# facebookresearch/momentum

Measured on NVIDIA H100. Metric: GN iterations/sec (batched 72-joint IK), higher is better.
Workload: dtype f32

## Files before the change

momentum_b200/csrc/ik_chol_sched.cuh:

```cuda
#pragma once

#include <cmath>
#include <cstring>

#include "ik_types.h"

#include <vector_types.h>

namespace mb2 {

struct CholSchedDev {
  int32_t n, nPad, numTileCols, numTiles, numLevels;
  const int32_t* blob;
  int32_t blobInts;
  const int32_t* perm;
  const int32_t* pos;
  const int32_t* tileIdTable;
  const int32_t* tileRow;
  const int32_t* tileCol;
  const int32_t* diagTile;
  const int32_t* levelColStart;
  const int32_t* levelCols;
  const int32_t* levelPanelStart;
  const int32_t* panelTile;
  const int32_t* panelDiag;
  const int32_t* levelTaskStart;
  const int32_t* taskDst;
  const int32_t* taskPairStart;
  const int32_t* pairA;
  const int32_t* pairB;
  const int32_t* levelVTaskStart;
  const int32_t* vtaskRow;
  const int32_t* vtaskSrcStart;
  const int32_t* vsrcTile;
  const int32_t* vsrcCol;
  const int32_t* colPanelStart;
  const int32_t* colPanelTile;
  const int32_t* colPanelRow;
  const int32_t* levelOrderStart8;
  const int32_t* taskOrder8;
  const int32_t* levelOrderStart16;
  const int32_t* taskOrder16;
  const int32_t* tileInfo;
};
MB2_HD CholSchedDev rebaseSchedule(const CholSchedDev& S, const int32_t* newBlob) {
  CholSchedDev R = S;
  const int32_t* o = S.blob;
  R.blob = newBlob;
#define MB2_RB(f) R.f = newBlob + (S.f - o);
  MB2_RB(perm) MB2_RB(pos) MB2_RB(tileIdTable) MB2_RB(tileRow) MB2_RB(tileCol) MB2_RB(diagTile) MB2_RB(levelColStart) MB2_RB(levelCols)
  MB2_RB(levelPanelStart) MB2_RB(panelTile) MB2_RB(panelDiag) MB2_RB(levelTaskStart) MB2_RB(taskDst) MB2_RB(taskPairStart) MB2_RB(pairA) MB2_RB(pairB)
  MB2_RB(levelVTaskStart) MB2_RB(vtaskRow) MB2_RB(vtaskSrcStart) MB2_RB(vsrcTile) MB2_RB(vsrcCol) MB2_RB(colPanelStart) MB2_RB(colPanelTile)
  MB2_RB(colPanelRow) MB2_RB(levelOrderStart8) MB2_RB(taskOrder8) MB2_RB(levelOrderStart16) MB2_RB(taskOrder16) MB2_RB(tileInfo)
#undef MB2_RB
  return R;
}

MB2_HD int tileSlotOffset(int lane) { return (lane ^ (lane >> 3)) << 2; }
MB2_HD int tileIdx(int r, int c) {
  const int lane = ((r & 7) << 2) | ((c & 7) >> 1);
  return ((c >> 3) << 7) + ((lane ^ (lane >> 3)) << 2) + (((r >> 3) << 1) | (c & 1));
}
MB2_HD int fragRow(int lane, int e) { return (lane >> 2) + 8 * (e >> 1); }
MB2_HD int fragCol(int lane, int h, int e) { return 8 * h + 2 * (lane & 3) + (e & 1); }
MB2_HD void tileLoadFrag(const float* tile, int lane, float d[2][4]) {
  const int so = tileSlotOffset(lane);
#if defined(__CUDA_ARCH__)
  const float4 v0 = *reinterpret_cast<const float4*>(tile + so), v1 = *reinterpret_cast<const float4*>(tile + 128 + so);
  d[0][0] = v0.x; d[0][1] = v0.y; d[0][2] = v0.z; d[0][3] = v0.w; d[1][0] = v1.x; d[1][1] = v1.y; d[1][2] = v1.z; d[1][3] = v1.w;
#else
  for (int h = 0; h < 2; ++h) for (int e = 0; e < 4; ++e) d[h][e] = tile[128 * h + so + e];
#endif
}
MB2_HD void tileStoreFrag(float* tile, int lane, const float d[2][4]) {
  const int so = tileSlotOffset(lane);
#if defined(__CUDA_ARCH__)
  *reinterpret_cast<float4*>(tile + so) = make_float4(d[0][0], d[0][1], d[0][2], d[0][3]);
  *reinterpret_cast<float4*>(tile + 128 + so) = make_float4(d[1][0], d[1][1], d[1][2], d[1][3]);
#else
  for (int h = 0; h < 2; ++h) for (int e = 0; e < 4; ++e) tile[128 * h + so + e] = d[h][e];
#endif
}

MB2_HD float cholPadElement(float v, int info, int r, int c) {
  const int vI = info & 0xFF, vJ = (info >> 8) & 0xFF, diag = (info >> 16) & 1;
  if (r < vI && c < vJ) return v;
  return (diag && r == c) ? 1.f : 0.f;
}
MB2_HD int tmaBoxIdx(int c, int r) { return c * 16 + ((((r >> 2) ^ ((c >> 1) & 3)) << 2) | (r & 3)); }
MB2_HD void cholConvertBox(float* tile, int info, int lane) {
  float v[2][4];
#pragma unroll
  for (int h = 0; h < 2; ++h)
#pragma unroll
    for (int e = 0; e < 4; ++e) {
      const int r = fragRow(lane, e), c = fragCol(lane, h, e);
      const bool mirror = ((info >> 16) & 1) != 0 && c > r;
      v[h][e] = cholPadElement(tile[mirror ? tmaBoxIdx(r, c) : tmaBoxIdx(c, r)], info, r, c);
    }
#if defined(__CUDA_ARCH__)
  __syncwarp();
#endif
  tileStoreFrag(tile, lane, v);
}

MB2_HD float tf32High(float x) {
#if defined(__CUDA_ARCH__)
  return __uint_as_float((__float_as_uint(x) + 0x1000u) & 0xFFFFE000u);
#else
  uint32_t u;
  std::memcpy(&u, &x, 4);
  u = (u + 0x1000u) & 0xFFFFE000u;
  float r;
  std::memcpy(&r, &u, 4);
  return r;
#endif
}
#if defined(__CUDA_ARCH__)
__device__ __forceinline__ void mmaTf32K8(float d[4], float a0, float a1, float a2, float a3, float b0, float b1) {
  asm volatile("mma.sync.aligned.m16n8k8.row.col.f32.tf32.tf32.f32 {%0, %1, %2, %3}, {%4, %5, %6, %7}, {%8, %9}, {%0, %1, %2, %3};"
               : "+f"(d[0]), "+f"(d[1]), "+f"(d[2]), "+f"(d[3])
               : "r"(__float_as_uint(a0)), "r"(__float_as_uint(a1)), "r"(__float_as_uint(a2)), "r"(__float_as_uint(a3)), "r"(__float_as_uint(b0)),
                 "r"(__float_as_uint(b1)));
}
__device__ __forceinline__ void mma3xTf32Step(float d[2][4], float small[2][4], float a0, float a1, float a2, float a3, float b00, float b01, float b10, float b11) {
  const float a0h = tf32High(a0), a1h = tf32High(a1), a2h = tf32High(a2), a3h = tf32High(a3);
  const float b00h = tf32High(b00), b01h = tf32High(b01), b10h = tf32High(b10), b11h = tf32High(b11);
  const float a0l = a0 - a0h, a1l = a1 - a1h, a2l = a2 - a2h, a3l = a3 - a3h;
  const float b00l = b00 - b00h, b01l = b01 - b01h, b10l = b10 - b10h, b11l = b11 - b11h;
  mmaTf32K8(small[0], a0l, a1l, a2l, a3l, b00h, b01h); mmaTf32K8(small[1], a0l, a1l, a2l, a3l, b10h, b11h);
  mmaTf32K8(small[0], a0h, a1h, a2h, a3h, b00l, b01l); mmaTf32K8(small[1], a0h, a1h, a2h, a3h, b10l, b11l);
  float t0[4] = {0.f, 0.f, 0.f, 0.f}, t1[4] = {0.f, 0.f, 0.f, 0.f};
  mmaTf32K8(t0, a0h, a1h, a2h, a3h, b00h, b01h); mmaTf32K8(t1, a0h, a1h, a2h, a3h, b10h, b11h);
#pragma unroll
  for (int e = 0; e < 4; ++e) { d[0][e] += t0[e]; d[1][e] += t1[e]; }
}
#endif
MB2_HD void mma3xEmulate(float& d, float& small, const float av[8], const float bv[8]) {
  float lo = 0.f, mid = 0.f, hi = 0.f;
  for (int k = 0; k < 8; ++k) {
    const float ah = tf32High(av[k]), bh = tf32High(bv[k]), al = av[k] - ah, bl = bv[k] - bh;
    lo += al * bh; mid += ah * bl; hi += ah * bh;
  }
  small += lo + mid;
  d += hi;
}

MB2_HD void gramTilePairs(const float* strips, int oa0, int ob0, int oa1, int ob1, int lane, float d[2][4], float small[2][4]) {
  const float* A0 = strips + oa0;
  const float* B0 = strips + ob0;
  const float* A1 = strips + oa1;
  const float* B1 = strips + ob1;
#if defined(__CUDA_ARCH__)
  mma3xTf32Step(d, small, A0[lane], A0[32 + lane], A1[lane], A1[32 + lane], B0[lane], B1[lane], B0[32 + lane], B1[32 + lane]);
#else
  for (int h = 0; h < 2; ++h)
    for (int e = 0; e < 4; ++e) {
      const int r = fragRow(lane, e), c = fragCol(lane, h, e);
      float av[8], bv[8];
      for (int k = 0; k < 8; ++k) { av[k] = k < 4 ? A0[4 * r + k] : A1[4 * r + k - 4]; bv[k] = k < 4 ? B0[4 * c + k] : B1[4 * c + k - 4]; }
      mma3xEmulate(d[h][e], small[h][e], av, bv);
    }
#endif
}
MB2_HD int4 tableRecord4(const int32_t* p) {
#if defined(__CUDA_ARCH__)
  return *reinterpret_cast<const int4*>(p);
#else
  int4 r; r.x = p[0]; r.y = p[1]; r.z = p[2]; r.w = p[3];
  return r;
#endif
}
MB2_HD int4 tableRecord4(const uint16_t* p) {
  int4 r;
#if defined(__CUDA_ARCH__)
  const uint2 v = *reinterpret_cast<const uint2*>(p);
  r.x = int(v.x & 0xFFFFu); r.y = int(v.x >> 16); r.z = int(v.y & 0xFFFFu); r.w = int(v.y >> 16);
#else
  r.x = p[0]; r.y = p[1]; r.z = p[2]; r.w = p[3];
#endif
  return r;
}
MB2_HD int2 tableRecord2(const uint16_t* p) {
  int2 r;
#if defined(__CUDA_ARCH__)
  const uint32_t v = *reinterpret_cast<const uint32_t*>(p);
  r.x = int(v & 0xFFFFu); r.y = int(v >> 16);
#else
  r.x = p[0]; r.y = p[1];
#endif
  return r;
}
template <class Q>
MB2_HD void gramTileAccumulate(const float* strips, const Q* quads, int q0, int q1, int lane, float d[2][4]) {
  float small[2][4] = {{0.f, 0.f, 0.f, 0.f}, {0.f, 0.f, 0.f, 0.f}};
  for (int q = q0; q < q1; ++q) {
    const int4 o = tableRecord4(quads + 4 * q);
    gramTilePairs(strips, o.x, o.y, o.z, o.w, lane, d, small);
  }
#pragma unroll
  for (int h = 0; h < 2; ++h)
#pragma unroll
    for (int e = 0; e < 4; ++e) d[h][e] += small[h][e];
}
MB2_HD void gramTileStore(float* tile, const float d[2][4], int info, float lambda, int lane) {
  const int vI = info & 0xFF, vJ = (info >> 8) & 0xFF, diag = (info >> 16) & 1;
  if (vI == 16 && vJ == 16 && !diag) { tileStoreFrag(tile, lane, d); return; }
  float v[2][4];
#pragma unroll
  for (int h = 0; h < 2; ++h)
#pragma unroll
    for (int e = 0; e < 4; ++e) {
      const int r = fragRow(lane, e), c = fragCol(lane, h, e);
      v[h][e] = cholPadElement((diag && r == c) ? d[h][e] + lambda : d[h][e], info, r, c);
    }
  tileStoreFrag(tile, lane, v);
}
MB2_HD void gramVectorTerm(const float* strip, const float* r4, int hl, float& g0, float& g1) {
  const float4 sv = *reinterpret_cast<const float4*>(strip + 4 * hl);
  const float4 rv = *reinterpret_cast<const float4*>(r4);
  g0 += sv.x * rv.x + sv.y * rv.y;
  g1 += sv.z * rv.z + sv.w * rv.w;
}
MB2_HD float gramVectorEntry(const float* strips, const float* resid, const int32_t* colStrip, const int32_t* stripRow, int s0, int s1, int hl) {
  float g0 = 0.f, g1 = 0.f;
  for (int k = s0; k < s1; ++k) {
    const int sidx = colStrip[k];
    gramVectorTerm(strips + size_t(sidx) * 64, resid + stripRow[sidx], hl, g0, g1);
  }
  return g0 + g1;
}
MB2_HD float gramVectorEntry(const float* strips, const float* resid, const uint16_t* colEnt, int s0, int s1, int hl) {
  float g0 = 0.f, g1 = 0.f;
  for (int k = s0; k < s1; ++k) {
    const int2 e = tableRecord2(colEnt + 2 * k);
    gramVectorTerm(strips + e.x, resid + e.y, hl, g0, g1);
  }
  return g0 + g1;
}

MB2_HD void tileLoadRow(const float* tile, int r, float* a) {
#pragma unroll
  for (int j = 0; j < 16; j += 2) {
    const float2 v = *reinterpret_cast<const float2*>(tile + tileIdx(r, j));
    a[j] = v.x; a[j + 1] = v.y;
  }
}
MB2_HD void tileStoreRow(float* tile, int r, const float* a) {
#pragma unroll
  for (int j = 0; j < 16; j += 2) {
    float2 v;
    v.x = a[j]; v.y = a[j + 1];
    *reinterpret_cast<float2*>(tile + tileIdx(r, j)) = v;
  }
}

MB2_HD void cholDiagTile(float* tile, float* y16, int lane, float fallback, int* fail) {
#if defined(__CUDA_ARCH__)
  const int hl = lane & 15;
  const bool isE = lane >= 16;
  float v[16];
#pragma unroll
  for (int k = 0; k < 16; ++k) v[k] = isE ? (k == hl ? 1.f : 0.f) : tile[tileIdx(k, hl)];
  float z = isE ? 0.f : y16[hl], rdSelf = 0.f;
  __syncwarp();
#pragma unroll
  for (int k = 0; k < 16; ++k) {
    float* blk = tile + 32 * (k & 1);
    if (!isE) { blk[hl] = v[k]; blk[16 + hl] = z; }
    __syncwarp();
    float c[16];
#pragma unroll
    for (int g4 = (k >> 2); g4 < 4; ++g4) {
      const float4 q = *reinterpret_cast<const float4*>(blk + 4 * g4);
      c[4 * g4] = q.x; c[4 * g4 + 1] = q.y; c[4 * g4 + 2] = q.z; c[4 * g4 + 3] = q.w;
    }
    float piv = c[k];
    const float zk = blk[16 + k];
    if (!(piv > 0.f)) { piv = fallback; if (lane == k) *fail = 1; }
    float inv;
    asm("rcp.approx.ftz.f32 %0, %1;" : "=f"(inv) : "f"(piv));
    const float rdk = rsqrtf(piv);
    if (lane == k) rdSelf = rdk;
    const float m = v[k] * inv;
    const float tm = (!isE && hl > k) ? m : 0.f;
#pragma unroll
    for (int j = k + 1; j < 16; ++j) v[j] -= m * c[j];
    z -= tm * zk;
    v[k] *= rdk;
  }
  __syncwarp();
  if (!isE) y16[hl] = z * rdSelf;
  else {
#pragma unroll
    for (int i = 0; i < 16; ++i) tile[tileIdx(i, hl)] = v[i];
  }
#else
  if (lane != 0) return;
  float A[16][16], E[16][16], z[16], rd[16];
  for (int l = 0; l < 16; ++l) { for (int k = 0; k < 16; ++k) { A[l][k] = tile[tileIdx(k, l)]; E[k][l] = (k == l) ? 1.f : 0.f; } z[l] = y16[l]; }
  for (int k = 0; k < 16; ++k) {
    float piv = A[k][k];
    if (!(piv > 0.f)) { piv = fallback; *fail = 1; }
    const float inv = 1.f / piv;
    rd[k] = 1.f / sqrtf(piv);
    const float zk = z[k];
    float c[16];
    for (int j = 0; j < 16; ++j) c[j] = A[j][k];
    for (int l = 0; l < 16; ++l) {
      const float m = c[l] * inv;
      for (int j = k + 1; j < 16; ++j) A[l][j] -= m * c[j];
      if (l > k) z[l] -= m * zk;
    }
    for (int l = 0; l < 16; ++l) {
      const float m = E[k][l] * inv;
      for (int j = k + 1; j < 16; ++j) E[j][l] -= m * c[j];
      E[k][l] *= rd[k];
    }
  }
  for (int l = 0; l < 16; ++l) {
    y16[l] = z[l] * rd[l];
    for (int i = 0; i < 16; ++i) tile[tileIdx(i, l)] = E[i][l];
  }
#endif
}

MB2_HD void tileProduct(const float* TA, const float* TB, int lane, float d[2][4], float small[2][4]) {
#if defined(__CUDA_ARCH__)
  const int so = tileSlotOffset(lane);
  const float4 a0 = *reinterpret_cast<const float4*>(TA + so), a1 = *reinterpret_cast<const float4*>(TA + 128 + so);
  const float4 b0 = *reinterpret_cast<const float4*>(TB + so), b1 = *reinterpret_cast<const float4*>(TB + 128 + so);
  mma3xTf32Step(d, small, a0.x, a0.z, a0.y, a0.w, b0.x, b0.y, b0.z, b0.w);
  mma3xTf32Step(d, small, a1.x, a1.z, a1.y, a1.w, b1.x, b1.y, b1.z, b1.w);
#else
  for (int h = 0; h < 2; ++h)
    for (int e = 0; e < 4; ++e) {
      const int r = fragRow(lane, e), c = fragCol(lane, h, e);
      for (int ks = 0; ks < 2; ++ks) {
        float av[8], bv[8];
        for (int k = 0; k < 8; ++k) { av[k] = TA[tileIdx(r, 8 * ks + k)]; bv[k] = TB[tileIdx(c, 8 * ks + k)]; }
        mma3xEmulate(d[h][e], small[h][e], av, bv);
      }
    }
#endif
}

MB2_HD void cholPanelProduct(const float* tile, const float* diagW, int lane, float out[2][4]) {
  float small[2][4];
#pragma unroll
  for (int h = 0; h < 2; ++h)
#pragma unroll
    for (int e = 0; e < 4; ++e) { out[h][e] = 0.f; small[h][e] = 0.f; }
  tileProduct(tile, diagW, lane, out, small);
#pragma unroll
  for (int h = 0; h < 2; ++h)
#pragma unroll
    for (int e = 0; e < 4; ++e) out[h][e] += small[h][e];
}
MB2_HD void cholPanelStore(float* tile, int lane, const float out[2][4]) { tileStoreFrag(tile, lane, out); }

template <class I>
MB2_HD void cholUpdateTile(float* tiles, const I* pairA, const I* pairB, int stride, int p0, int p1, int dst, int lane) {
  float d[2][4], small[2][4];
#pragma unroll
  for (int h = 0; h < 2; ++h)
#pragma unroll
    for (int e = 0; e < 4; ++e) { d[h][e] = 0.f; small[h][e] = 0.f; }
  for (int p = p0; p < p1; ++p)
    tileProduct(tiles + size_t(pairA[p * stride]) * 256, tiles + size_t(pairB[p * stride]) * 256, lane, d, small);
  float* D = tiles + size_t(dst) * 256;
  float v[2][4];
  tileLoadFrag(D, lane, v);
#pragma unroll
  for (int h = 0; h < 2; ++h)
#pragma unroll
    for (int e = 0; e < 4; ++e) v[h][e] -= d[h][e] + small[h][e];
  tileStoreFrag(D, lane, v);
}
MB2_HD void cholUpdateTask(float* tiles, const CholSchedDev& S, int task, int lane) {
  cholUpdateTile(tiles, S.pairA, S.pairB, 1, S.taskPairStart[task], S.taskPairStart[task + 1], S.taskDst[task], lane);
}

template <class I>
MB2_HD void cholVectorRows(const float* tiles, float* y, const I* srcTile, const I* srcCol, int stride, int p0, int p1, int row, int hl) {
  float s0 = 0.f, s1 = 0.f, s2 = 0.f, s3 = 0.f;
  for (int p = p0; p < p1; ++p) {
    float t[16];
    tileLoadRow(tiles + size_t(srcTile[p * stride]) * 256, hl, t);
    const float* yk = y + srcCol[p * stride] * 16;
#pragma unroll
    for (int c = 0; c < 16; c += 4) { s0 += t[c] * yk[c]; s1 += t[c + 1] * yk[c + 1]; s2 += t[c + 2] * yk[c + 2]; s3 += t[c + 3] * yk[c + 3]; }
  }
  y[row * 16 + hl] -= (s0 + s1) + (s2 + s3);
}
MB2_HD void cholVectorTask(const float* tiles, float* y, const CholSchedDev& S, int vtask, int hl) {
  cholVectorRows(tiles, y, S.vsrcTile, S.vsrcCol, 1, S.vtaskSrcStart[vtask], S.vtaskSrcStart[vtask + 1], S.vtaskRow[vtask], hl);
}

template <class I>
MB2_HD void cholBackwardPanels(const float* tiles, float* y, const I* panelTile, const I* panelRow, int stride, int p0, int p1, int K, int diag, int lane) {
#if defined(__CUDA_ARCH__)
  const int g = lane >> 2, t = lane & 3, so = tileSlotOffset(lane);
  float c0 = 0.f, c1 = 0.f, c2 = 0.f, c3 = 0.f;
  for (int p = p0; p < p1; ++p) {
    const float* T = tiles + size_t(panelTile[p * stride]) * 256;
    const float* yi = y + panelRow[p * stride] * 16;
    const float4 v0 = *reinterpret_cast<const float4*>(T + so), v1 = *reinterpret_cast<const float4*>(T + 128 + so);
    const float ya = yi[g], yb = yi[g + 8];
    c0 = fmaf(v0.x, ya, fmaf(v0.z, yb, c0)); c1 = fmaf(v0.y, ya, fmaf(v0.w, yb, c1));
    c2 = fmaf(v1.x, ya, fmaf(v1.z, yb, c2)); c3 = fmaf(v1.y, ya, fmaf(v1.w, yb, c3));
  }
#pragma unroll
  for (int o = 4; o < 32; o <<= 1) {
    c0 += __shfl_xor_sync(0xffffffffu, c0, o); c1 += __shfl_xor_sync(0xffffffffu, c1, o);
    c2 += __shfl_xor_sync(0xffffffffu, c2, o); c3 += __shfl_xor_sync(0xffffffffu, c3, o);
  }
  float* yk = y + K * 16;
  if (g == 0) { yk[2 * t] -= c0; yk[2 * t + 1] -= c1; yk[8 + 2 * t] -= c2; yk[9 + 2 * t] -= c3; }
  __syncwarp();
  const float* W = tiles + size_t(diag) * 256;
  const float4 w0 = *reinterpret_cast<const float4*>(W + so), w1 = *reinterpret_cast<const float4*>(W + 128 + so);
  const float sa = yk[g], sb = yk[g + 8];
  float x0 = fmaf(w0.x, sa, w0.z * sb), x1 = fmaf(w0.y, sa, w0.w * sb), x2 = fmaf(w1.x, sa, w1.z * sb), x3 = fmaf(w1.y, sa, w1.w * sb);
#pragma unroll
  for (int o = 4; o < 32; o <<= 1) {
    x0 += __shfl_xor_sync(0xffffffffu, x0, o); x1 += __shfl_xor_sync(0xffffffffu, x1, o);
    x2 += __shfl_xor_sync(0xffffffffu, x2, o); x3 += __shfl_xor_sync(0xffffffffu, x3, o);
  }
  __syncwarp();
  if (g == 0) { yk[2 * t] = x0; yk[2 * t + 1] = x1; yk[8 + 2 * t] = x2; yk[9 + 2 * t] = x3; }
#else
  if (lane != 0) return;
  float s[16];
  for (int c = 0; c < 16; ++c) s[c] = 0.f;
  for (int p = p0; p < p1; ++p) {
    const float* T = tiles + size_t(panelTile[p * stride]) * 256;
    const float* yi = y + panelRow[p * stride] * 16;
    for (int c = 0; c < 16; ++c) for (int r = 0; r < 16; ++r) s[c] += T[tileIdx(r, c)] * yi[r];
  }
  float* yk = y + K * 16;
  for (int c = 0; c < 16; ++c) s[c] = yk[c] - s[c];
  const float* W = tiles + size_t(diag) * 256;
  for (int c = 0; c < 16; ++c) {
    float x = 0.f;
    for (int r = 0; r < 16; ++r) x += W[tileIdx(r, c)] * s[r];
    yk[c] = x;
  }
#endif
}
MB2_HD void cholBackwardColumn(const float* tiles, float* y, const CholSchedDev& S, int K, int lane) {
  cholBackwardPanels(tiles, y, S.colPanelTile, S.colPanelRow, 1, S.colPanelStart[K], S.colPanelStart[K + 1], K, S.diagTile[K], lane);
}

}
```

momentum_b200/csrc/ik_kernels.cu:

```cuda
#include "ik_kernels.cuh"

#include <algorithm>
#include <cstdio>
#include <type_traits>

#include "ik_chol.cuh"
#include "ik_chol_sched.h"
#include "ik_jtj_tc.cuh"
#include "ik_ptx.cuh"
#include "ik_device.cuh"
#include "ik_jacobi.cuh"

namespace mb2 {

__device__ __forceinline__ double warpSum(double v) {
  for (int o = 16; o > 0; o >>= 1) v += __shfl_xor_sync(0xffffffffu, v, o);
  return v;
}

size_t sweepSmemPerInstance(const FunctionTables& T, int warpsPerInstance) {
  const size_t nPad = (T.numParams + 3) & ~3;
  const size_t jp = warpsPerInstance > 1 ? size_t((T.numJoints * kParametersPerJoint + 1) & ~1) : 0;
  return sizeof(float) * (nPad + jp + size_t((T.numJoints * kJointStateStride + 1) & ~1) + size_t((T.recStride + 1) & ~1) + 4 + 2 * size_t(warpsPerInstance));
}
// ... 961 lines not shown
  extern __shared__ float smem[];
  const int b = blockIdx.x;
  if (a.active[b] == 0) return;
  const int n = a.ns;
  const int tid = threadIdx.x;
  float* Hg = a.H + size_t(b) * a.hStride;
  CholCtx ctx;
  ctx.n = n;
  int ldp = ((n + 1 + 3) & ~3) + 4;
  float* P = smem;
  float* gsave = P + NB * ldp;
  int* flags = reinterpret_cast<int*>(gsave + ((n + 3) & ~3));
  float* As = reinterpret_cast<float*>(flags + 4);
  if (useSmemMatrix) {
    ctx.lda = n | 1;
    ctx.A = As;
    for (int idx = tid; idx < (n + 1) * n; idx += kCholThreads) {
      const int j = idx / (n + 1), i = idx - j * (n + 1);
      if (i >= j) {
        float v = Hg[size_t(j) * a.ldH + i];
        if (i == j) v += a.regularization;
        As[i * ctx.lda + j] = v;
      }
    }
  } else {
    ctx.lda = a.ldH;
    ctx.A = Hg;
    for (int idx = tid; idx < (n + 1) * n; idx += kCholThreads) {
      const int j = idx / (n + 1), i = idx - j * (n + 1);
      if (i > j) Hg[size_t(i) * a.ldH + j] = Hg[size_t(j) * a.ldH + i];
    }
    for (int i = tid; i < n; i += kCholThreads) Hg[size_t(i) * a.ldH + i] += a.regularization;
  }
  ctx.P = P;
  ctx.ldp = ldp;
  ctx.fail = flags;
  if (tid == 0) flags[0] = 0;
  for (int i = tid; i < n; i += kCholThreads) gsave[i] = Hg[size_t(i) * a.ldH + n];
  __syncthreads();

  const int blockSize = cholBlockSize(n, NB);
  for (int k = 0; k < n; k += blockSize) {
    const int bs = min(blockSize, n - k);
    if (tid < 32) {
      for (int jj = 0; jj < bs; ++jj) {
        const float x = cholDiagPivot(ctx, k, jj);
        __syncwarp();
        if (!(x > 0.f)) { if (tid == 0) flags[0] = k + jj + 1; break; }
        cholDiagColumn(ctx, k, bs, jj, x, tid);
        __syncwarp();
      }
    }
    __syncthreads();
    if (flags[0] != 0) break;
    cholPanelSolve<NB>(ctx, k, bs, tid, kCholThreads);
    __syncthreads();
    cholTrailingUpdate<NB>(ctx, k, bs, tid, kCholThreads);
    __syncthreads();
  }
  float* y = ctx.A + size_t(n) * ctx.lda;
  if (flags[0] != 0) {
    if (tid == 0) cholForwardFrom(ctx, cholCompletedColumns(flags[0] - 1, blockSize), y);
    __syncthreads();
  }
  for (int i0 = ((n - 1) / 32) * 32; i0 >= 0; i0 -= 32) {
    const int nb = min(32, n - i0);
    if (tid < 32) {
      float yv = tid < nb ? y[i0 + tid] : 0.f;
      float dinv = tid < nb ? 1.f / ctx.A[size_t(i0 + tid) * ctx.lda + i0 + tid] : 0.f;
      for (int kk = nb - 1; kk >= 0; --kk) {
        const float xk = __shfl_sync(0xffffffffu, yv, kk) * __shfl_sync(0xffffffffu, dinv, kk);
        if (tid == kk) yv = xk;
        else if (tid < kk) yv -= ctx.A[size_t(i0 + kk) * ctx.lda + i0 + tid] * xk;
      }
      if (tid < nb) y[i0 + tid] = yv;
    }
    __syncthreads();
    for (int i = tid; i < i0; i += kCholThreads) {
      float s = y[i];
      for (int kk = 0; kk < nb; ++kk) s -= ctx.A[size_t(i0 + kk) * ctx.lda + i] * y[i0 + kk];
      y[i] = s;
    }
    __syncthreads();
  }
  cholFinish(a, b, n, y, gsave, flags[0] != 0);
}

cudaError_t launchCholesky(const CholArgs& a, int NB, bool inSmem, cudaStream_t stream) {
  const size_t smem = cholSmemBytes(a.ns, NB, inSmem);
  if (NB != 8 && NB != 16 && NB != 32) return cudaErrorInvalidConfiguration;
  cudaError_t e = cudaSuccess;
#define MB2_LAUNCH_CHOL(NBV)                                                                                   \
  e = cudaFuncSetAttribute(choleskyKernel<NBV>, cudaFuncAttributeMaxDynamicSharedMemorySize, int(smem));       \
  if (e != cudaSuccess) return e;                                                                              \
  choleskyKernel<NBV><<<a.batch, kCholThreads, smem, stream>>>(a, inSmem ? 1 : 0);
  if (NB == 8) { MB2_LAUNCH_CHOL(8) } else if (NB == 16) { MB2_LAUNCH_CHOL(16) } else { MB2_LAUNCH_CHOL(32) }
#undef MB2_LAUNCH_CHOL
  return cudaGetLastError();
}

constexpr int kGramThreads = 32 * kGramWarps;

template <int kThreads>
__global__ void __launch_bounds__(kThreads) gramTilesKernel(const GramArgs a) {
  extern __shared__ __align__(16) float gramSmem[];
  const int b = blockIdx.x;
  if (a.active != nullptr && a.active[b] == 0) return;
  const int tid = threadIdx.x, warp = tid >> 5, lane = tid & 31, hw = tid >> 4, hl = tid & 15;
  float* strips = gramSmem + (((128u - (smemAddr(gramSmem) & 127u)) & 127u) >> 2);
  float* resid = strips + a.residOff;
  float* zero = strips + a.stripStride;
  unsigned long long* bar = reinterpret_cast<unsigned long long*>(zero + 64);
  const uint32_t barAddr = smemAddr(bar);
  const uint32_t total = uint32_t(a.stripStride) * 4u;
  if (tid < 64) zero[tid] = 0.f;
  if (tid == 0) {
    mbarInit(barAddr, 1);
    fenceBarrierInit();
    mbarExpectTx(barAddr, total);
    const char* src = reinterpret_cast<const char*>(a.strips + size_t(b) * a.stripStride);
    for (uint32_t off = 0; off < total; off += 16384u) bulkLoad(smemAddr(strips) + off, src + off, total - off < 16384u ? total - off : 16384u, barAddr);
  }
  int32_t* tab = reinterpret_cast<int32_t*>(bar + 2);
  for (int i = tid; i < a.blobInts; i += kThreads) tab[i] = __ldg(a.blob + i);
  __syncthreads();
  mbarWaitRelaxed(barAddr, 0);
  const int32_t* tileOrder = tab + a.offTileOrder, *tileQuadStart = tab + a.offTilePairStart, *quads = tab + a.offPairA;
  const int32_t* colStripStart = tab + a.offColStripStart, *colStrip = tab + a.offColStrip, *stripRow = tab + a.offStripRow, *tileInfo = tab + a.offTileInfo;
  float* out = a.out + size_t(b) * a.outStride;
  for (int ti = warp; ti < a.numOrder; ti += kThreads / 32) {
    const int t = tileOrder[ti];
    if (t < 0) continue;
    float acc[2][4];
#pragma unroll
    for (int i = 0; i < 2; ++i)
#pragma unroll
      for (int j = 0; j < 4; ++j) acc[i][j] = 0.f;
    gramTileAccumulate(strips, quads, tileQuadStart[t], tileQuadStart[t + 1], lane, acc);
    gramTileStore(out + size_t(t) * 256, acc, tileInfo[t], a.regularization, lane);
  }
  float* y = out + size_t(a.numTiles) * 256;
  for (int K = hw; K < a.numTileCols; K += kThreads / 16)
    y[16 * K + hl] = gramVectorEntry(strips, resid, colStrip, stripRow, colStripStart[K], colStripStart[K + 1], hl);
}

cudaError_t launchGramTiles(const GramArgs& a, int threads, cudaStream_t stream) {
  const size_t smem = gramTilesSmemBytes(a.stripStride, a.blobInts);
  if (smem > size_t(g_maxSmemOptin) || (a.stripStride & 3) != 0 || (threads != 256 && threads != 512)) return cudaErrorInvalidConfiguration;
  const bool wide = threads == 512;
  cudaError_t e = wide ? cudaFuncSetAttribute(gramTilesKernel<512>, cudaFuncAttributeMaxDynamicSharedMemorySize, int(smem))
                       : cudaFuncSetAttribute(gramTilesKernel<kGramThreads>, cudaFuncAttributeMaxDynamicSharedMemorySize, int(smem));
  if (e != cudaSuccess) return e;
  if (wide) gramTilesKernel<512><<<a.batch, 512, smem, stream>>>(a);
  else gramTilesKernel<kGramThreads><<<a.batch, kGramThreads, smem, stream>>>(a);
  return cudaGetLastError();
}


template <int kSchedThreads, bool kProfile>
__global__ void __launch_bounds__(kSchedThreads, kSchedThreads == 256 ? 3 : 1) choleskyScheduledKernel(const __grid_constant__ CUtensorMap hmap, const CholArgs a, const CholSchedDev Sg) {
  extern __shared__ __align__(16) float smemRaw[];
  const int b = blockIdx.x;
  if (a.active[b] == 0) return;
  const int n = a.ns, tid = threadIdx.x;
  const int warp = tid >> 5, lane = tid & 31, hw = tid >> 4, hl = tid & 15;
  const unsigned hmask = 0xFFFFu << (16 * ((tid >> 4) & 1));
  float* tiles = smemRaw + (((1024u - (smemAddr(smemRaw) & 1023u)) & 1023u) >> 2);
  float* y = tiles + size_t(Sg.numTiles) * 256;
  float* gsub = y + Sg.nPad;
  float* dsub = gsub + ((n + 3) & ~3);
  int32_t* blob = reinterpret_cast<int32_t*>(dsub + ((n + 3) & ~3));
  int* flags = reinterpret_cast<int*>(blob + ((Sg.blobInts + 3) & ~3));
  unsigned long long* bar = reinterpret_cast<unsigned long long*>(flags + 2);
  long long pc[9] = {0, 0, 0, 0, 0, 0, 0, 0, 0}, pt = clock64();
#define MB2_PROF(k) if constexpr (kProfile) { const long long now = clock64(); pc[k] += now - pt; pt = now; }
  const uint32_t barAddr = smemAddr(bar);
  const uint32_t blobBytes = uint32_t((Sg.blobInts + 3) & ~3) * 4u, gBytes = uint32_t(a.ldG) * 4u;
  const bool fromGram = a.tilesIn != nullptr;
  const uint32_t tileBytes = uint32_t(Sg.numTiles) * 1024u, yBytes = uint32_t(Sg.nPad) * 4u;
  if (tid == 0) {
    flags[0] = 0;
    mbarInit(barAddr, 1);
    fenceBarrierInit();
    mbarExpectTx(barAddr, blobBytes + tileBytes + (fromGram ? yBytes : gBytes));
  }
  __syncthreads();
  if (fromGram) {
    if (tid == 0) {
      bulkLoad(smemAddr(blob), Sg.blob, blobBytes, barAddr);
      const float* src = a.tilesIn + size_t(b) * a.tilesStride;
      const uint32_t total = tileBytes + yBytes;
      for (uint32_t off = 0; off < total; off += 16384u)
        bulkLoad(smemAddr(tiles) + off, reinterpret_cast<const char*>(src) + off, total - off < 16384u ? total - off : 16384u, barAddr);
    }
  } else {
    if (tid == 0) {
      bulkLoad(smemAddr(blob), Sg.blob, blobBytes, barAddr);
      bulkLoad(smemAddr(gsub), a.g + size_t(b) * a.ldG, gBytes, barAddr);
    }
    for (int t = tid; t < Sg.numTiles; t += kSchedThreads) {
      const int gi0 = __ldg(Sg.tileInfo + 3 * t), gj0 = __ldg(Sg.tileInfo + 3 * t + 1);
      tmaLoad3d(smemAddr(tiles + size_t(t) * 256), &hmap, gi0, gj0, b, barAddr);
    }
  }
  MB2_PROF(6)
  mbarWaitRelaxed(barAddr, 0);
  MB2_PROF(7)
  const CholSchedDev S = rebaseSchedule(Sg, blob);
  if (fromGram) {
    for (int s = tid; s < S.nPad; s += kSchedThreads) {
      const int p = S.perm[s];
      if (p >= 0) gsub[p] = y[s];
    }
  } else {
    for (int t = warp; t < S.numTiles; t += kSchedThreads / 32) cholConvertBox(tiles + size_t(t) * 256, S.tileInfo[3 * t + 2], lane);
    for (int s = tid; s < S.nPad; s += kSchedThreads) {
      const int p = S.perm[s];
      y[s] = p >= 0 ? gsub[p] : 0.f;
    }
  }
  __syncthreads();
  MB2_PROF(8)
  if (!fromGram)
    for (int s = tid; s < S.nPad; s += kSchedThreads)
      if (S.perm[s] >= 0) tiles[size_t(S.diagTile[s >> 4]) * 256 + tileIdx(s & 15, s & 15)] += a.regularization;
  __syncthreads();
  MB2_PROF(0)

  for (int L = 0; L < S.numLevels; ++L) {
    for (int ci = S.levelColStart[L] + warp; ci < S.levelColStart[L + 1]; ci += kSchedThreads / 32) {
      const int K = S.levelCols[ci];
      cholDiagTile(tiles + size_t(S.diagTile[K]) * 256, y + 16 * K, lane, a.regularization, flags);
    }
    __syncthreads();
    MB2_PROF(1)
    for (int pi = S.levelPanelStart[L] + warp; pi < S.levelPanelStart[L + 1]; pi += kSchedThreads / 32) {
      float* ptile = tiles + size_t(S.panelTile[pi]) * 256;
      float x[2][4];
      cholPanelProduct(ptile, tiles + size_t(S.panelDiag[pi]) * 256, lane, x);
      cholPanelStore(ptile, lane, x);
    }
    __syncthreads();
    MB2_PROF(2)
    {
      const int32_t* oStart = kSchedThreads == 256 ? S.levelOrderStart8 : S.levelOrderStart16, *order = kSchedThreads == 256 ? S.taskOrder8 : S.taskOrder16;
      for (int oi = oStart[L] + warp; oi < oStart[L + 1]; oi += kSchedThreads / 32) { const int ti = order[oi]; if (ti >= 0) cholUpdateTask(tiles, S, ti, lane); }
    }
    for (int vi = S.levelVTaskStart[L] + hw; vi < S.levelVTaskStart[L + 1]; vi += kSchedThreads / 16) cholVectorTask(tiles, y, S, vi, hl);
    __syncthreads();
    MB2_PROF(3)
  }
  for (int L = S.numLevels - 1; L >= 0; --L) {
    for (int ci = S.levelColStart[L] + warp; ci < S.levelColStart[L + 1]; ci += kSchedThreads / 32) cholBackwardColumn(tiles, y, S, S.levelCols[ci], lane);
    __syncthreads();
  }
  MB2_PROF(4)
  for (int i = tid; i < S.nPad; i += kSchedThreads) { const int p = S.perm[i]; if (p >= 0) dsub[p] = y[i]; }
  __syncthreads();
  cholFinish(a, b, n, dsub, gsub, flags[0] != 0);
  MB2_PROF(5)
  if (kProfile && b == 0 && tid == 0)
    printf("chol-profile (cycles, block 0): blob %lld issue %lld wait %lld lambda %lld diag %lld panel %lld update %lld backward %lld finish %lld | levels %d tiles %d\n", pc[6], pc[7],
           pc[8], pc[0], pc[1], pc[2], pc[3], pc[4], pc[5], S.numLevels, S.numTiles);
#undef MB2_PROF
}

cudaError_t launchCholeskyScheduled(const CholArgs& a, const CholSchedDev& sched, int threads, cudaStream_t stream) {
  const size_t smem = choleskyScheduledSmemBytes(a.ns, sched.nPad, sched.numTiles, sched.blobInts);
  if (smem > size_t(g_maxSmemOptin) || (threads != 256 && threads != 512)) return cudaErrorInvalidConfiguration;
  const bool wide = threads == 512;
  const bool prof = (a.profile & 1) != 0;
  cudaError_t e;
  if (wide) e = prof ? cudaFuncSetAttribute(choleskyScheduledKernel<512, true>, cudaFuncAttributeMaxDynamicSharedMemorySize, int(smem))
                     : cudaFuncSetAttribute(choleskyScheduledKernel<512, false>, cudaFuncAttributeMaxDynamicSharedMemorySize, int(smem));
  else e = prof ? cudaFuncSetAttribute(choleskyScheduledKernel<256, true>, cudaFuncAttributeMaxDynamicSharedMemorySize, int(smem))
                : cudaFuncSetAttribute(choleskyScheduledKernel<256, false>, cudaFuncAttributeMaxDynamicSharedMemorySize, int(smem));
  if (e != cudaSuccess) return e;
  if (a.tilesIn == nullptr && (a.g == nullptr || a.ldG != cholGradientLd(a.ns))) return cudaErrorInvalidValue;
  if ((a.ldH & 3) != 0 || (a.hStride & 3) != 0 || (a.tilesStride & 3) != 0) return cudaErrorInvalidValue;
  CUtensorMap hmap;
  const bool fromGram = a.tilesIn != nullptr;
  const uint64_t dims[3] = {uint64_t(fromGram ? 256 : a.ldH), uint64_t(fromGram ? sched.numTiles : a.ns + 1), uint64_t(a.batch)};
  const uint64_t strides[2] = {uint64_t(fromGram ? 256 : a.ldH) * sizeof(float), uint64_t(fromGram ? a.tilesStride : a.hStride) * sizeof(float)};
  const uint32_t box[3] = {16u, 16u, 1u};
  e = makeTensorMap3d(&hmap, fromGram ? a.tilesIn : a.H, dims, strides, box, 64);
  if (e != cudaSuccess) return e;
  if (wide && prof) choleskyScheduledKernel<512, true><<<a.batch, 512, smem, stream>>>(hmap, a, sched);
  else if (wide) choleskyScheduledKernel<512, false><<<a.batch, 512, smem, stream>>>(hmap, a, sched);
  else if (prof) choleskyScheduledKernel<256, true><<<a.batch, 256, smem, stream>>>(hmap, a, sched);
  else choleskyScheduledKernel<256, false><<<a.batch, 256, smem, stream>>>(hmap, a, sched);
  return cudaGetLastError();
}

__device__ int acquireParkSlot(uint32_t* words, int numWords, int start) {
  for (int w = start % numWords;; w = (w + 1 == numWords) ? 0 : w + 1) {
    uint32_t freeBits = ~__ldcg(words + w);
    while (freeBits != 0u) {
      const int bit = __ffs(freeBits) - 1;
      if ((atomicOr(words + w, 1u << bit) & (1u << bit)) == 0u) return 32 * w + bit;
      freeBits &= freeBits - 1u;
    }
  }
}

template <bool kProfile, class Tables>
__global__ void __launch_bounds__(kGramThreads, 4) gramCholeskyKernel(const GramCholArgs a, const CholSchedDev S, const __grid_constant__ Tables P) {
  extern __shared__ __align__(16) float gcSmem[];
  const GramArgs& g = a.g;
  const CholArgs& c = a.c;
  const int b = blockIdx.x;
  if (c.active[b] == 0) return;
  const int n = c.ns, tid = threadIdx.x;
  const int warp = tid >> 5, lane = tid & 31, hw = tid >> 4, hl = tid & 15;
  constexpr int kWarps = kGramThreads / 32;
  float* U = gcSmem + (((128u - (smemAddr(gcSmem) & 127u)) & 127u) >> 2);
  const size_t tileFloats = size_t(S.numTiles) * 256, sweepFloats = g.stripStride + 64;
  const size_t uni = ((tileFloats > sweepFloats ? tileFloats : sweepFloats) + 3) & ~size_t(3);
  float* strips = U;
  float* resid = U + g.residOff;
  float* tiles = U;
  float* y = U + uni;
  float* gsub = y + S.nPad;
  int* flags = reinterpret_cast<int*>(gsub + ((n + 3) & ~3));
  unsigned long long* bar = reinterpret_cast<unsigned long long*>(flags + 4);
  const uint16_t* tab = P.tab;
  const GramCholLayout& L = P.L;
  long long pc[8] = {0, 0, 0, 0, 0, 0, 0, 0}, pt = 0;
  if constexpr (kProfile) pt = clock64();
#define MB2_GC(k) if constexpr (kProfile) { const long long now = clock64(); pc[k] += now - pt; pt = now; }
  const uint32_t barAddr = smemAddr(bar);
  const uint32_t stripBytes = uint32_t(g.stripStride) * 4u;
  if (tid == 0) {
    flags[0] = 0;
    mbarInit(barAddr, 1);
    fenceBarrierInit();
    mbarExpectTx(barAddr, stripBytes);
    const char* src = reinterpret_cast<const char*>(g.strips + size_t(b) * g.stripStride);
    for (uint32_t off = 0; off < stripBytes; off += 16384u) bulkLoad(smemAddr(strips) + off, src + off, stripBytes - off < 16384u ? stripBytes - off : 16384u, barAddr);
    flags[1] = a.parkTiles > 0 ? acquireParkSlot(a.parkSlots, a.parkSlotWords, b) : 0;
  }
  if (tid >= 64 && tid < 128) strips[g.stripStride + (tid - 64)] = 0.f;
  __syncthreads();
  mbarWaitRelaxed(barAddr, 0);
  MB2_GC(0)
  float* park = a.park + size_t(flags[1]) * size_t(a.parkTiles) * 256 + 4 * lane;
  const int rounds = g.numOrder / kWarps;
  auto tileInfoOf = [](int packed) { return (packed & 0x7FFF) | ((packed >> 15) << 16); };
  for (int r = 0; r < rounds; ++r) {
    const int4 rec = tableRecord4(tab + L.gram + 4 * (r * kWarps + warp));
    if (rec.x == 0xFFFF) continue;
    float acc[2][4];
#pragma unroll
    for (int i = 0; i < 2; ++i)
#pragma unroll
      for (int j = 0; j < 4; ++j) acc[i][j] = 0.f;
    gramTileAccumulate(strips, tab + L.quad, rec.z, rec.w, lane, acc);
    if (rec.x >= a.parkTiles) gramTileStore(tiles + size_t(rec.x) * 256, acc, tileInfoOf(rec.y), g.regularization, lane);
    else {
      __stcg(reinterpret_cast<float4*>(park + size_t(rec.x) * 256), make_float4(acc[0][0], acc[0][1], acc[0][2], acc[0][3]));
      __stcg(reinterpret_cast<float4*>(park + size_t(rec.x) * 256 + 128), make_float4(acc[1][0], acc[1][1], acc[1][2], acc[1][3]));
    }
  }
  for (int K = hw; K < S.numTileCols; K += kGramThreads / 16)
    y[16 * K + hl] = gramVectorEntry(strips, resid, tab + L.colEnt, int(tab[L.col + K]), int(tab[L.col + K + 1]), hl);
  __syncthreads();
  MB2_GC(1)
  for (int r = 0; r < rounds; ++r) {
    const int4 rec = tableRecord4(tab + L.gram + 4 * (r * kWarps + warp));
    if (rec.x == 0xFFFF || rec.x >= a.parkTiles) continue;
    const float4 v0 = __ldcg(reinterpret_cast<const float4*>(park + size_t(rec.x) * 256));
    const float4 v1 = __ldcg(reinterpret_cast<const float4*>(park + size_t(rec.x) * 256 + 128));
    const float acc[2][4] = {{v0.x, v0.y, v0.z, v0.w}, {v1.x, v1.y, v1.z, v1.w}};
    gramTileStore(tiles + size_t(rec.x) * 256, acc, tileInfoOf(rec.y), g.regularization, lane);
  }
  for (int s2 = tid; s2 < S.nPad; s2 += kGramThreads) {
    const int p = S.perm[s2];
    if (p >= 0) gsub[p] = y[s2];
  }
  __syncthreads();
  if (tid == 0 && a.parkTiles > 0) atomicAnd(a.parkSlots + (flags[1] >> 5), ~(1u << (flags[1] & 31)));
  MB2_GC(2)
  for (int Lv = 0; Lv < S.numLevels; ++Lv) {
    const int4 l0 = tableRecord4(tab + L.level + 4 * Lv), l1 = tableRecord4(tab + L.level + 4 * (Lv + 1));
    for (int ci = l0.x + warp; ci < l1.x; ci += kWarps) {
      const int4 d = tableRecord4(tab + L.diag + 4 * ci);
      cholDiagTile(tiles + size_t(d.y) * 256, y + 16 * d.x, lane, c.regularization, flags);
    }
    __syncthreads();
    MB2_GC(3)
    for (int pi = l0.y + warp; pi < l1.y; pi += kWarps) {
      const int2 pe = tableRecord2(tab + L.panel + 2 * pi);
      float* ptile = tiles + size_t(pe.x) * 256;
      float x[2][4];
      cholPanelProduct(ptile, tiles + size_t(pe.y) * 256, lane, x);
      cholPanelStore(ptile, lane, x);
    }
    __syncthreads();
    MB2_GC(4)
    for (int oi = l0.z + warp; oi < l1.z; oi += kWarps) {
      const int4 o = tableRecord4(tab + L.order + 4 * oi);
      if (o.x != 0xFFFF) cholUpdateTile(tiles, tab + L.pair, tab + L.pair + 1, 2, o.y, o.z, o.x, lane);
    }
    for (int vi = l0.w + hw; vi < l1.w; vi += kGramThreads / 16) {
      const int4 v = tableRecord4(tab + L.vtask + 4 * vi);
      cholVectorRows(tiles, y, tab + L.vsrc, tab + L.vsrc + 1, 2, v.y, v.z, v.x, hl);
    }
    __syncthreads();
    MB2_GC(5)
  }
  for (int Lv = S.numLevels - 1; Lv >= 0; --Lv) {
    const int c0 = tab[L.level + 4 * Lv], c1 = tab[L.level + 4 * (Lv + 1)];
    for (int ci = c0 + warp; ci < c1; ci += kWarps) {
      const int4 d = tableRecord4(tab + L.diag + 4 * ci);
      cholBackwardPanels(tiles, y, tab + L.colPanel, tab + L.colPanel + 1, 2, d.z, d.w, d.x, d.y, lane);
    }
    __syncthreads();
  }
  MB2_GC(6)
  cholFinish(c, b, n, y, gsub, flags[0] != 0, S.pos);
  MB2_GC(7)
  if constexpr (kProfile) {
    if (b == int(gridDim.x >> 1) && tid == 0 && a.phaseCycles != nullptr)
      for (int k = 0; k < 8; ++k) a.phaseCycles[k] += (unsigned long long)pc[k];
  }
#undef MB2_GC
}

template <bool kProfile, class Tables>
static cudaError_t prepareGramCholesky(size_t smem) {
  cudaError_t e = cudaFuncSetAttribute(gramCholeskyKernel<kProfile, Tables>, cudaFuncAttributeMaxDynamicSharedMemorySize, int(smem));
  if (e != cudaSuccess) return e;
  return cudaFuncSetAttribute(gramCholeskyKernel<kProfile, Tables>, cudaFuncAttributePreferredSharedMemoryCarveout, int(cudaSharedmemCarveoutMaxShared));
}

int gramCholeskyParkSlots(const GramCholArgs& a, const CholSchedDev& sched, bool paramTables) {
  const size_t smem = gramCholeskySmemBytes(a.g.stripStride, a.c.ns, sched.nPad, sched.numTiles);
  cudaError_t e = paramTables ? prepareGramCholesky<false, GramCholParamTables>(smem) : prepareGramCholesky<false, GramCholGlobalTables>(smem);
  int perSm = 0;
  if (e == cudaSuccess)
    e = paramTables ? cudaOccupancyMaxActiveBlocksPerMultiprocessor(&perSm, gramCholeskyKernel<false, GramCholParamTables>, kGramThreads, smem)
                    : cudaOccupancyMaxActiveBlocksPerMultiprocessor(&perSm, gramCholeskyKernel<false, GramCholGlobalTables>, kGramThreads, smem);
  if (e != cudaSuccess || perSm < 1) return -1;
  return (g_numSms * perSm + 31) / 32 * 32;
}

cudaError_t launchGramCholesky(const GramCholArgs& a, const CholSchedDev& sched, const GramCholParamTables* inParams, const GramCholGlobalTables& inGlobal, bool profile,
                               cudaStream_t stream) {
  const size_t smem = gramCholeskySmemBytes(a.g.stripStride, a.c.ns, sched.nPad, sched.numTiles);
  if (smem > size_t(g_maxSmemOptin) || (a.g.stripStride & 3) != 0) return cudaErrorInvalidConfiguration;
  if (a.parkTiles > 0 && (a.park == nullptr || a.parkSlots == nullptr || a.parkSlotWords < 1)) return cudaErrorInvalidValue;
  cudaError_t e;
  if (inParams != nullptr) e = profile ? prepareGramCholesky<true, GramCholParamTables>(smem) : prepareGramCholesky<false, GramCholParamTables>(smem);
  else e = profile ? prepareGramCholesky<true, GramCholGlobalTables>(smem) : prepareGramCholesky<false, GramCholGlobalTables>(smem);
  if (e != cudaSuccess) return e;
  if (inParams != nullptr) {
    if (profile) gramCholeskyKernel<true, GramCholParamTables><<<a.c.batch, kGramThreads, smem, stream>>>(a, sched, *inParams);
    else gramCholeskyKernel<false, GramCholParamTables><<<a.c.batch, kGramThreads, smem, stream>>>(a, sched, *inParams);
  } else {
    if (profile) gramCholeskyKernel<true, GramCholGlobalTables><<<a.c.batch, kGramThreads, smem, stream>>>(a, sched, inGlobal);
    else gramCholeskyKernel<false, GramCholGlobalTables><<<a.c.batch, kGramThreads, smem, stream>>>(a, sched, inGlobal);
  }
  return cudaGetLastError();
}

}
#include "ik_qr.cuh"
#include "ik_tr_qr.cuh"
namespace mb2 {

cudaError_t initKernelAttributes() {
  int dev = 0;
  cudaError_t e = cudaGetDevice(&dev);
  if (e != cudaSuccess) return e;
  e = cudaDeviceGetAttribute(&g_numSms, cudaDevAttrMultiProcessorCount, dev);
  if (e != cudaSuccess) return e;
  e = cudaDeviceGetAttribute(&g_maxSmemPerSm, cudaDevAttrMaxSharedMemoryPerMultiprocessor, dev);
  if (e != cudaSuccess) return e;
  return cudaDeviceGetAttribute(&g_maxSmemOptin, cudaDevAttrMaxSharedMemoryPerBlockOptin, dev);
}

__global__ void trialUpdateKernel(int batch, const float* thetaOrig, int ldTheta, const float* delta, int ns, const int32_t* cols, const float* scale,
                                  float* thetaTrial, const int32_t* active) {
  const int b = blockIdx.x;
  if (active[b] == 0) return;
  const float s = scale[b];
  for (int i = threadIdx.x; i < ns; i += blockDim.x) {
    const int c = cols[i];
    if (c >= 0) thetaTrial[size_t(b) * ldTheta + c] = thetaOrig[size_t(b) * ldTheta + c] - s * delta[size_t(b) * ns + i];
  }
}
cudaError_t launchTrialUpdate(int batch, const float* thetaOrig, int ldTheta, const float* delta, int ns, const int32_t* cols, const float* scale,
                              float* thetaTrial, const int32_t* active, cudaStream_t stream) {
  trialUpdateKernel<<<batch, 128, 0, stream>>>(batch, thetaOrig, ldTheta, delta, ns, cols, scale, thetaTrial, active);
  return cudaGetLastError();
}

__global__ void lineSearchStepKernel(const LineSearchArgs a) {
  const int b = blockIdx.x * blockDim.x + threadIdx.x;
  if (b >= a.batch || a.searching[b] == 0) return;
  const double error = a.errors[b], errorNew = a.trialErrors[b];
  const float scale = a.scale[b];
  bool accept;
  if (!a.subsetVariant) {
    const float scaledError = 1e-3f * (float)error;
    accept = (error - errorNew) >= (double)(scale * scaledError);
  } else {
    accept = (error - errorNew) >= (double)(1e-4f * scale) * (double)a.gradDotDelta[b];
  }
  if (accept || a.step >= 9) a.searching[b] = 0;
  else a.scale[b] = scale * 0.5f;
}
cudaError_t launchLineSearchStep(const LineSearchArgs& a, cudaStream_t stream) {
  lineSearchStepKernel<<<(a.batch + 127) / 128, 128, 0, stream>>>(a);
  return cudaGetLastError();
}

__global__ void commitTrialKernel(int batch, int numParams, int ldTheta, const float* thetaTrial, float* theta, const int32_t* active) {
  const int b = blockIdx.x;
  if (active[b] == 0) return;
  for (int i = threadIdx.x; i < numParams; i += blockDim.x) theta[size_t(b) * ldTheta + i] = thetaTrial[size_t(b) * ldTheta + i];
}
cudaError_t launchCommitTrial(int batch, int numParams, int ldTheta, const float* thetaTrial, float* theta, const int32_t* active, cudaStream_t stream) {
  commitTrialKernel<<<batch, 128, 0, stream>>>(batch, numParams, ldTheta, thetaTrial, theta, active);
  return cudaGetLastError();
}

__global__ void bookkeepingKernel(const BookkeepingArgs a) {
  const int b = blockIdx.x * blockDim.x + threadIdx.x;
  if (b >= a.batch || a.active[b] == 0) return;
  const double error = a.errors[b], last = a.lastErrors[b];
  if (a.history != nullptr) a.history[size_t(b) * a.maxIterations + a.iteration] = error;
  const bool converged = fabs(last - error) / (fabs(error) + (double)FLT_MIN) <= (double)(a.threshold * FLT_EPSILON);
  a.iterations[b] = a.iteration + 1;
  if ((a.iteration >= a.minIterations && converged) || a.iteration + 1 >= a.maxIterations) a.active[b] = 0;
  else { a.lastErrors[b] = error; atomicAdd(a.activeCount, 1); }
}
cudaError_t launchBookkeeping(const BookkeepingArgs& a, cudaStream_t stream) {
  bookkeepingKernel<<<(a.batch + 127) / 128, 128, 0, stream>>>(a);
  return cudaGetLastError();
}

__global__ void normalizeQuatsKernel(float* base, int count, int strideFloats, int quatsPerRecord, int batch) {
  const int idx = blockIdx.x * blockDim.x + threadIdx.x;
  if (idx >= batch * quatsPerRecord) return;
  const int b = idx / quatsPerRecord, q = idx % quatsPerRecord;
  float* p = base + size_t(b) * strideFloats + 4 * q;
  const float n = sqrtf(p[0] * p[0] + p[1] * p[1] + p[2] * p[2] + p[3] * p[3]);
  p[0] /= n; p[1] /= n; p[2] /= n; p[3] /= n;
}
__global__ void scatterTargetsKernel(const float* packed, float* dst, int size, int strideFloats, int batch) {
  const size_t idx = size_t(blockIdx.x) * blockDim.x + threadIdx.x;
  if (idx >= size_t(batch) * size) return;
  const size_t b = idx / size, k = idx % size;
  dst[b * strideFloats + k] = packed[idx];
}
cudaError_t launchScatterTargets(const float* packed, float* dst, int size, int strideFloats, int batch, cudaStream_t stream) {
  const size_t total = size_t(batch) * size;
  if (total == 0) return cudaSuccess;
  scatterTargetsKernel<<<unsigned((total + 255) / 256), 256, 0, stream>>>(packed, dst, size, strideFloats, batch);
  return cudaGetLastError();
}
cudaError_t launchNormalizeQuats(float* base, int count, int strideFloats, int quatsPerRecord, int batch, cudaStream_t stream) {
  const int total = batch * quatsPerRecord;
  if (total == 0) return cudaSuccess;
  normalizeQuatsKernel<<<(total + 127) / 128, 128, 0, stream>>>(base, count, strideFloats, quatsPerRecord, batch);
  return cudaGetLastError();
}

DeviceLimits deviceLimits() { return DeviceLimits{g_numSms, g_maxSmemOptin, g_maxSmemPerSm}; }

}
```

momentum_b200/csrc/ik_ptx.cuh:

```cuda
#pragma once

#include <cuda.h>

#include <cstdint>
#include <cstdio>

namespace mb2 {

constexpr unsigned long long kSpinLimit = 4000000000ull;

__device__ __forceinline__ uint32_t smemAddr(const void* p) { return static_cast<uint32_t>(__cvta_generic_to_shared(p)); }

__device__ __forceinline__ void mbarInit(uint32_t bar, uint32_t count) {
  asm volatile("mbarrier.init.shared::cta.b64 [%0], %1;" ::"r"(bar), "r"(count) : "memory");
}
__device__ __forceinline__ void mbarExpectTx(uint32_t bar, uint32_t bytes) {
  asm volatile("mbarrier.arrive.expect_tx.shared::cta.b64 _, [%0], %1;" ::"r"(bar), "r"(bytes) : "memory");
}
__device__ __forceinline__ void mbarArrive(uint32_t bar) {
  asm volatile("mbarrier.arrive.shared::cta.b64 _, [%0];" ::"r"(bar) : "memory");
}
__device__ __forceinline__ void mbarWait(uint32_t bar, uint32_t parity) {
  uint32_t done = 0;
  const long long t0 = clock64();
  while (true) {
    asm volatile(
        "{\n\t.reg .pred p;\n\t"
        "mbarrier.try_wait.parity.shared::cta.b64 p, [%1], %2;\n\t"
        "selp.u32 %0, 1, 0, p;\n\t}"
        : "=r"(done)
        : "r"(bar), "r"(parity)
        : "memory");
    if (done) break;
    if ((uint64_t)(clock64() - t0) > kSpinLimit) {
      printf("momentum_b200: mbarrier timeout (block %d thread %d bar %u parity %u)\n", blockIdx.x, threadIdx.x, bar, parity);
      __trap();
    }
  }
}
template <bool kSleep>
__device__ __forceinline__ void mbarWaitSilent(uint32_t bar, uint32_t parity) {
  uint32_t done = 0;
  const long long t0 = clock64();
  while (true) {
    asm volatile(
        "{\n\t.reg .pred p;\n\t"
        "mbarrier.try_wait.parity.shared::cta.b64 p, [%1], %2;\n\t"
        "selp.u32 %0, 1, 0, p;\n\t}"
        : "=r"(done)
        : "r"(bar), "r"(parity)
        : "memory");
    if (done) break;
    if constexpr (kSleep) __nanosleep(32);
    if ((uint64_t)(clock64() - t0) > kSpinLimit) __trap();
  }
}
__device__ __forceinline__ void mbarWaitRelaxed(uint32_t bar, uint32_t parity) {
  uint32_t done = 0;
  const long long t0 = clock64();
  while (true) {
    asm volatile(
        "{\n\t.reg .pred p;\n\t"
        "mbarrier.try_wait.parity.shared::cta.b64 p, [%1], %2;\n\t"
        "selp.u32 %0, 1, 0, p;\n\t}"
        : "=r"(done)
        : "r"(bar), "r"(parity)
        : "memory");
    if (done) break;
    __nanosleep(32);
    if ((uint64_t)(clock64() - t0) > kSpinLimit) {
      printf("momentum_b200: mbarrier timeout (block %d thread %d bar %u parity %u)\n", blockIdx.x, threadIdx.x, bar, parity);
      __trap();
    }
  }
}
__device__ __forceinline__ void tmaLoad3d(uint32_t dst, const CUtensorMap* map, int c0, int c1, int c2, uint32_t bar) {
  asm volatile(
      "cp.async.bulk.tensor.3d.shared::cluster.global.tile.mbarrier::complete_tx::bytes [%0], [%1, {%2, %3, %4}], [%5];" ::"r"(dst),
      "l"(reinterpret_cast<uint64_t>(map)), "r"(c0), "r"(c1), "r"(c2), "r"(bar)
      : "memory");
}
__device__ __forceinline__ void bulkLoad(uint32_t dst, const void* src, uint32_t bytes, uint32_t bar) {
  asm volatile("cp.async.bulk.shared::cluster.global.mbarrier::complete_tx::bytes [%0], [%1], %2, [%3];" ::"r"(dst), "l"(src), "r"(bytes), "r"(bar) : "memory");
}
__device__ __forceinline__ void fenceBarrierInit() { asm volatile("fence.mbarrier_init.release.cluster;" ::: "memory"); }
__device__ __forceinline__ void fenceProxyAsync() { asm volatile("fence.proxy.async.shared::cta;" ::: "memory"); }

}
```

Before: 9.698 million.

## Park finished gram tiles in tile layout and reload them with bulk async copy

Gram tiles that spill to the global park buffer are now finalised (regularisation and padding applied) before parking and written in the shared tile layout. After the barrier they come back with a single bulk asynchronous copy tracked by an mbarrier, replacing a per-warp __ldcg reload and store loop. Acquiring the park slot moves off thread 0's critical path to the last warp, and consumers spin on a volatile flag only when they actually need to park. The change adds proxy fences and a second mbarrier phase, and relies on tileSlotOffset matching the in-shared layout.

```diff
diff --git a/momentum_b200/csrc/ik_chol_sched.cuh b/momentum_b200/csrc/ik_chol_sched.cuh
--- a/momentum_b200/csrc/ik_chol_sched.cuh
+++ b/momentum_b200/csrc/ik_chol_sched.cuh
@@ -203,17 +203,24 @@
 #pragma unroll
     for (int e = 0; e < 4; ++e) d[h][e] += small[h][e];
 }
-MB2_HD void gramTileStore(float* tile, const float d[2][4], int info, float lambda, int lane) {
+MB2_HD void gramTileFinish(float d[2][4], int info, float lambda, int lane) {
   const int vI = info & 0xFF, vJ = (info >> 8) & 0xFF, diag = (info >> 16) & 1;
-  if (vI == 16 && vJ == 16 && !diag) { tileStoreFrag(tile, lane, d); return; }
-  float v[2][4];
+  if (vI == 16 && vJ == 16 && !diag) return;
 #pragma unroll
   for (int h = 0; h < 2; ++h)
 #pragma unroll
     for (int e = 0; e < 4; ++e) {
       const int r = fragRow(lane, e), c = fragCol(lane, h, e);
-      v[h][e] = cholPadElement((diag && r == c) ? d[h][e] + lambda : d[h][e], info, r, c);
-    }
+      d[h][e] = cholPadElement((diag && r == c) ? d[h][e] + lambda : d[h][e], info, r, c);
+    }
+}
+MB2_HD void gramTileStore(float* tile, const float d[2][4], int info, float lambda, int lane) {
+  float v[2][4];
+#pragma unroll
+  for (int h = 0; h < 2; ++h)
+#pragma unroll
+    for (int e = 0; e < 4; ++e) v[h][e] = d[h][e];
+  gramTileFinish(v, info, lambda, lane);
   tileStoreFrag(tile, lane, v);
 }
 MB2_HD void gramVectorTerm(const float* strip, const float* r4, int hl, float& g0, float& g1) {
diff --git a/momentum_b200/csrc/ik_kernels.cu b/momentum_b200/csrc/ik_kernels.cu
--- a/momentum_b200/csrc/ik_kernels.cu
+++ b/momentum_b200/csrc/ik_kernels.cu
@@ -1287,6 +1287,11 @@
     }
   }
 }
+__device__ __forceinline__ int waitParkSlot(const int* flag) {
+  int slot;
+  while ((slot = *reinterpret_cast<const volatile int*>(flag)) < 0) {}
+  return slot;
+}
 
 template <bool kProfile, class Tables>
 __global__ void __launch_bounds__(kGramThreads, 4) gramCholeskyKernel(const GramCholArgs a, const CholSchedDev S, const __grid_constant__ Tables P) {
@@ -1317,20 +1322,21 @@
   const uint32_t stripBytes = uint32_t(g.stripStride) * 4u;
   if (tid == 0) {
     flags[0] = 0;
+    flags[1] = -1;
     mbarInit(barAddr, 1);
     fenceBarrierInit();
     mbarExpectTx(barAddr, stripBytes);
     const char* src = reinterpret_cast<const char*>(g.strips + size_t(b) * g.stripStride);
     for (uint32_t off = 0; off < stripBytes; off += 16384u) bulkLoad(smemAddr(strips) + off, src + off, stripBytes - off < 16384u ? stripBytes - off : 16384u, barAddr);
-    flags[1] = a.parkTiles > 0 ? acquireParkSlot(a.parkSlots, a.parkSlotWords, b) : 0;
   }
   if (tid >= 64 && tid < 128) strips[g.stripStride + (tid - 64)] = 0.f;
   __syncthreads();
+  if (tid == kGramThreads - 32 && a.parkTiles > 0) *reinterpret_cast<volatile int*>(flags + 1) = acquireParkSlot(a.parkSlots, a.parkSlotWords, b);
   mbarWaitRelaxed(barAddr, 0);
   MB2_GC(0)
-  float* park = a.park + size_t(flags[1]) * size_t(a.parkTiles) * 256 + 4 * lane;
   const int rounds = g.numOrder / kWarps;
   auto tileInfoOf = [](int packed) { return (packed & 0x7FFF) | ((packed >> 15) << 16); };
+  int slot = -1;
   for (int r = 0; r < rounds; ++r) {
     const int4 rec = tableRecord4(tab + L.gram + 4 * (r * kWarps + warp));
     if (rec.x == 0xFFFF) continue;
@@ -1340,28 +1346,31 @@
 #pragma unroll
       for (int j = 0; j < 4; ++j) acc[i][j] = 0.f;
     gramTileAccumulate(strips, tab + L.quad, rec.z, rec.w, lane, acc);
-    if (rec.x >= a.parkTiles) gramTileStore(tiles + size_t(rec.x) * 256, acc, tileInfoOf(rec.y), g.regularization, lane);
+    gramTileFinish(acc, tileInfoOf(rec.y), g.regularization, lane);
+    if (rec.x >= a.parkTiles) tileStoreFrag(tiles + size_t(rec.x) * 256, lane, acc);
     else {
-      __stcg(reinterpret_cast<float4*>(park + size_t(rec.x) * 256), make_float4(acc[0][0], acc[0][1], acc[0][2], acc[0][3]));
-      __stcg(reinterpret_cast<float4*>(park + size_t(rec.x) * 256 + 128), make_float4(acc[1][0], acc[1][1], acc[1][2], acc[1][3]));
+      if (slot < 0) slot = waitParkSlot(flags + 1);
+      float* dst = a.park + (size_t(slot) * size_t(a.parkTiles) + size_t(rec.x)) * 256 + tileSlotOffset(lane);
+      __stcg(reinterpret_cast<float4*>(dst), make_float4(acc[0][0], acc[0][1], acc[0][2], acc[0][3]));
+      __stcg(reinterpret_cast<float4*>(dst + 128), make_float4(acc[1][0], acc[1][1], acc[1][2], acc[1][3]));
     }
   }
   for (int K = hw; K < S.numTileCols; K += kGramThreads / 16)
     y[16 * K + hl] = gramVectorEntry(strips, resid, tab + L.colEnt, int(tab[L.col + K]), int(tab[L.col + K + 1]), hl);
+  if (a.parkTiles > 0) fenceProxyAsyncGlobalShared();
   __syncthreads();
   MB2_GC(1)
-  for (int r = 0; r < rounds; ++r) {
-    const int4 rec = tableRecord4(tab + L.gram + 4 * (r * kWarps + warp));
-    if (rec.x == 0xFFFF || rec.x >= a.parkTiles) continue;
-    const float4 v0 = __ldcg(reinterpret_cast<const float4*>(park + size_t(rec.x) * 256));
-    const float4 v1 = __ldcg(reinterpret_cast<const float4*>(park + size_t(rec.x) * 256 + 128));
-    const float acc[2][4] = {{v0.x, v0.y, v0.z, v0.w}, {v1.x, v1.y, v1.z, v1.w}};
-    gramTileStore(tiles + size_t(rec.x) * 256, acc, tileInfoOf(rec.y), g.regularization, lane);
+  if (tid == 0 && a.parkTiles > 0) {
+    const uint32_t parkBytes = uint32_t(a.parkTiles) * 1024u;
+    mbarExpectTx(barAddr, parkBytes);
+    const char* src = reinterpret_cast<const char*>(a.park + size_t(flags[1]) * size_t(a.parkTiles) * 256);
+    for (uint32_t off = 0; off < parkBytes; off += 16384u) bulkLoad(smemAddr(tiles) + off, src + off, parkBytes - off < 16384u ? parkBytes - off : 16384u, barAddr);
   }
   for (int s2 = tid; s2 < S.nPad; s2 += kGramThreads) {
     const int p = S.perm[s2];
     if (p >= 0) gsub[p] = y[s2];
   }
+  if (a.parkTiles > 0) mbarWaitSilent<false>(barAddr, 1);
   __syncthreads();
   if (tid == 0 && a.parkTiles > 0) atomicAnd(a.parkSlots + (flags[1] >> 5), ~(1u << (flags[1] & 31)));
   MB2_GC(2)
diff --git a/momentum_b200/csrc/ik_ptx.cuh b/momentum_b200/csrc/ik_ptx.cuh
--- a/momentum_b200/csrc/ik_ptx.cuh
+++ b/momentum_b200/csrc/ik_ptx.cuh
@@ -85,5 +85,8 @@
 }
 __device__ __forceinline__ void fenceBarrierInit() { asm volatile("fence.mbarrier_init.release.cluster;" ::: "memory"); }
 __device__ __forceinline__ void fenceProxyAsync() { asm volatile("fence.proxy.async.shared::cta;" ::: "memory"); }
+__device__ __forceinline__ void fenceProxyAsyncGlobalShared() {
+  asm volatile("fence.proxy.async.global;\n\tfence.proxy.async.shared::cta;" ::: "memory");
+}
 
 }
```

Result: faster. 9.969 million, median of 6 (+2.8%).
